# PacificBiosciences/trgt

Hardware: AMD Instinct MI355X
Metric: loci/s (higher is better)
Workload: dtype u8/u16 (WFA) + f64 (HMM); 1 GPU; BASELINE configs[1]: 10000 synthetic single-motif STR loci per GPU (motif 3-6 bp, allele <= 200 bp), 30 reads/locus HiFi-like, 10% truncated reads (SURVEY.md Appendix E), seed 20250509; contexts_per_gpu=4, loci_per_gpu=10000, reads_per_locus=30, parallelism=loci sharded across 1 GPU(s), no collective

## Files before the change

trgt_amd/csrc/common.hpp:

```cpp
#pragma once
#include <hip/hip_runtime.h>

#include <cstdarg>
#include <cstdint>
#include <cstdio>
#include <cstring>
#include <ctime>
#include <algorithm>
#include <mutex>
#include <string>
#include <vector>

#include "../../include/trgt_hip.h"

#ifdef TRGT_DEV_BUILD
#define TRGT_DEV_ENV(name) getenv(name)
#else
#define TRGT_DEV_ENV(name) ((const char*)nullptr)
#endif

struct trgt_knobs {
  int filter_force = 0;
  int flank_threads = 256;
  int heavy_band = 96;
  int heavy_threads = 0;
  int band_threads = 64;
  int win_threads = 64;
  int win_segments = 8;
  bool win_lds = false;
  int grid_per_cu = 0;
  int filter_per_cu = 0;
  bool one_launch = false;
  bool no_spec = false;
  bool no_window = false;
  bool early_adaptive = true;
  bool no_heavy_window = false;
  bool no_sibling_rule = false;
  bool no_settled_sibling_rule = false;
  bool no_lcs_rule = false;
  bool no_indel_shortcut = false;
  bool no_hamming = false;
  bool no_filter = false;
  bool one_stream = false;
  bool host_genotyper = false;
// ... 53 lines not shown
  uint64_t ws_limit = 32ull << 30;
  int32_t cluster_max_reads = 256;
  int32_t size_max_reads = 256;
  int64_t size_deep_stats[4] = {0, 0, 0, 0};
  bool flank_device = false;
  int64_t flank_stats[4] = {0, 0, 0, 0};
  bool snv_split_device = false;
  int64_t snv_split_stats[4] = {0, 0, 0, 0};
  bool flank_cluster_device = false;
  bool snv_cluster_device = false;
  int64_t snv_cluster_stats[4] = {0, 0, 0, 0};
  int64_t flank_cluster_stats[3] = {0, 0, 0};
  bool flank_cluster_deep_device = false;
  int64_t flank_cluster_deep_stats[3] = {0, 0, 0};
  int num_cus = 256;
  struct Buf { void* p = nullptr; size_t cap = 0; };
  std::vector<Buf> pool;
  bool timing = false;
  double k_ms[TRGT_K_COUNT] = {};
  int64_t k_launches[TRGT_K_COUNT] = {};
  int64_t k_cells[TRGT_K_COUNT] = {};
  struct Pending { int k; hipEvent_t a, b; };
  std::vector<Pending> pending;
  std::vector<hipEvent_t> retired_events;
  void* zero_arena = nullptr; size_t zero_cap = 0, zero_used = 0, zero_dirty = 0; bool zero_on = false;
  void* wfa_cells_cur[3] = {nullptr, nullptr, nullptr};
  void* last_wfa_cells_dev = nullptr;
  void* last_filter_cells_dev = nullptr;
  int64_t dbg_ns[8] = {0, 0, 0, 0, 0, 0, 0, 0};
  int64_t tl_t0 = 0;
// ... 115 lines not shown
  S_CL_VOUT, S_CL_VLEN, S_CL_VSCR,
  S_INF_SRC, S_INF_DESC, S_INF_DST, S_INF_STATUS, S_INF_COUNTER,
  S_ZERO_ARENA,
  S_DEFL_SCRATCH,
  S_PUR_SLAB, S_PUR_CNT, S_PUR_RQ,
  S_CLD_LIST, S_CLD_LAST = S_CLD_LIST + (S_CL_VSCR - S_CL_LIST),
  S_CLD_SEL,
  S_GSD_LIST,
  S_GT_HP,
  S_SNV_SO, S_SNV_EO, S_SNV_MM, S_SNV_MMOFF, S_SNV_READ,
  S_SNV_DEEP,
  S_CLF_COUNTS,
  S_CLF_PEND,
  S_CLDF_COUNTS, S_CLDF_PEND,
  S_FS_SETTLED, S_FS_FILTERJOBS,
  S_COUNT
};
enum PinSlot { P_SPAN_S = 0, P_SPAN_E, P_HIT_L, P_HIT_R, P_CELLS, P_HMM_SEQ, P_HMM_SEQ_B, P_HMM_JOBS, P_HMM_JOBS_B, P_SEG0, P_SEG_META, P_GT_NEED, P_GT_NAL, P_GT_ALEN, P_GT_CI, P_GT_NSP, P_GT_CLS,
               P_GT_RANK, P_GT_NSPAN, P_GT_TOFF, P_GT_PACKED, P_HMM_BUILD, P_PUR_JOBS, P_COUNT };

inline int dev_get(trgt_hip_ctx* c, int slot, size_t bytes, void** out) {
  if ((int)c->pool.size() < S_COUNT) c->pool.resize(S_COUNT);
  auto& b = c->pool[slot];
  if (bytes == 0) bytes = 16;
  if (b.cap < bytes) {
    if (b.p) { TRGT_HIP_TRY(c, hipFree(b.p)); b.p = nullptr; b.cap = 0; }
    size_t want = bytes + bytes / 8 + 256;
    if (c->knobs.debug && want > ((size_t)256 << 20)) fprintf(stderr, "[mem] slot %d: %.2f GB\n", slot, (double)want / (double)(1ull << 30));
    if (want >= ((size_t)64 << 20)) {
      size_t free_b = 0, total_b = 0;
// ... 298 lines not shown
```

trgt_amd/csrc/ctx.hip:

```cpp
#include "common.hpp"
#include "host_pool.hpp"

static std::string g_create_err;

#include <malloc.h>
static void tune_malloc_once() {
  static std::once_flag once;
  std::call_once(once, [] {
    const char* e = getenv("TRGT_MALLOC_TUNE");
    const int mode = e && *e ? atoi(e) : 1;
    if (mode <= 0) return;
    (void)mallopt(M_MMAP_THRESHOLD, 32 << 20);
    (void)mallopt(M_TRIM_THRESHOLD, 1 << 30);
    (void)mallopt(M_TOP_PAD, 64 << 20);
    if (mode >= 2) (void)mallopt(M_MMAP_MAX, 0);
  });
}

namespace trgt {
static thread_local int g_next_stream_priority = 0;
static thread_local bool g_next_in_pool = false;
void ctx_next_stream_priority(int p) { g_next_stream_priority = p; }
void ctx_next_in_pool(bool on) { g_next_in_pool = on; }
hipError_t make_stream(trgt_hip_ctx* c, hipStream_t* s) {
// ... 36 lines not shown
  tune_malloc_once();
  trgt_hip_ctx* c = new trgt_hip_ctx();
  {
    trgt_knobs& k = c->knobs;
    auto num = [](const char* name, int dflt) { const char* e = getenv(name); return e && *e ? atoi(e) : dflt; };
    auto flag = [](const char* name) { const char* e = getenv(name); return e != nullptr && *e != 0 && std::strcmp(e, "0") != 0; };
#ifdef TRGT_DEV_BUILD
#define DEV_FLAG(name) flag(name)
#define DEV_NUM(name, dflt) num(name, dflt)
#else
#define DEV_FLAG(name) false
#define DEV_NUM(name, dflt) (dflt)
#endif
    (void)num; (void)flag;
    k.flank_threads = DEV_NUM("TRGT_FLANK_THREADS", k.flank_threads); k.heavy_threads = DEV_NUM("TRGT_HEAVY_THREADS", 0); k.heavy_band = std::max(0, std::min(num("TRGT_HEAVY_BAND", k.heavy_band), 256));
    k.win_threads = DEV_NUM("TRGT_WIN_THREADS", k.win_threads); { const int bt = DEV_NUM("TRGT_BAND_THREADS", k.band_threads); k.band_threads = bt == 128 || bt == 256 ? bt : 64; } k.win_segments = DEV_NUM("TRGT_WIN_SEGMENTS", k.win_segments); k.win_lds = DEV_FLAG("TRGT_WIN_LDS");
    k.grid_per_cu = DEV_NUM("TRGT_WFA_GRID_PER_CU", 0); k.filter_per_cu = DEV_NUM("TRGT_FILTER_PER_CU", 0);
    k.one_launch = DEV_FLAG("TRGT_WFA_ONE_LAUNCH"); k.no_spec = DEV_FLAG("TRGT_WFA_NO_SPEC"); k.no_window = flag("TRGT_WFA_NO_WINDOW"); k.no_hamming = flag("TRGT_NO_HAMMING"); k.no_indel_shortcut = flag("TRGT_NO_INDEL_SHORTCUT"); k.no_heavy_window = DEV_FLAG("TRGT_NO_HEAVY_WINDOW"); k.no_sibling_rule = DEV_FLAG("TRGT_NO_SIBLING_RULE"); k.no_settled_sibling_rule = DEV_FLAG("TRGT_NO_SETTLED_SIBLING_RULE"); k.no_lcs_rule = DEV_FLAG("TRGT_NO_LCS_RULE"); { const char* e = TRGT_DEV_ENV("TRGT_EARLY_ADAPTIVE"); if (e && *e) k.early_adaptive = std::strcmp(e, "0") != 0; }
    k.no_filter = flag("TRGT_WFA_NO_FILTER"); k.one_stream = DEV_FLAG("TRGT_FLANK_ONE_STREAM"); k.host_genotyper = flag("TRGT_HOST_GENOTYPER"); k.host_hmm_lists = DEV_FLAG("TRGT_HOST_HMM_LISTS"); k.no_early = flag("TRGT_WFA_NO_EARLY"); k.stage_lock = flag("TRGT_STAGE_LOCK"); k.no_long_filter = flag("TRGT_NO_LONG_FILTER"); k.no_long_window = DEV_FLAG("TRGT_NO_LONG_WINDOW"); k.filter_force = DEV_NUM("TRGT_FILTER_FORCE", 0); k.filter_one_launch = DEV_FLAG("TRGT_FILTER_ONE_LAUNCH"); k.filter_serial = DEV_FLAG("TRGT_FILTER_SERIAL"); k.filter_side = DEV_FLAG("TRGT_FILTER_SIDE"); k.wfa_no_stage = DEV_FLAG("TRGT_WFA_NO_STAGE"); k.wfa_no_wave_variant = DEV_FLAG("TRGT_WFA_NO_WAVE_VARIANT"); k.hmm_resolve_one_wg = DEV_FLAG("TRGT_HMM_RESOLVE_ONE_WG"); k.debug = flag("TRGT_WFA_DEBUG");
    k.timeline = flag("TRGT_TIMELINE");
    k.host_repair = flag("TRGT_HOST_REPAIR"); k.host_cluster = flag("TRGT_HOST_CLUSTER"); k.host_purity = DEV_FLAG("TRGT_HOST_PURITY"); k.cluster_arena_kb = num("TRGT_CLUSTER_ARENA_KB", 0); k.repair_arena_kb = num("TRGT_REPAIR_ARENA_KB", 0); k.hmm_lds_fill = DEV_FLAG("TRGT_HMM_LDS_FILL"); k.hmm_four_rounds = DEV_FLAG("TRGT_HMM_FOUR_ROUNDS"); k.hmm_no_ppl = flag("TRGT_HMM_NO_PPL"); k.hmm_long_wgs = std::max(1, std::min(DEV_NUM("TRGT_HMM_LONG_WGS", k.hmm_long_wgs), 16)); k.hmm_no_long_tb = flag("TRGT_HMM_NO_LONG_TB"); k.hmm_no_dedupe = flag("TRGT_HMM_NO_DEDUPE"); k.repair_max_seg = num("TRGT_REPAIR_MAX_SEG", k.repair_max_seg); k.split_hmm = DEV_FLAG("TRGT_SPLIT_HMM"); k.repair_blocks = DEV_NUM("TRGT_REPAIR_BLOCKS", k.repair_blocks);
    k.no_lean = flag("TRGT_WFA_NO_LEAN"); k.lean_one_tier = DEV_FLAG("TRGT_WFA_LEAN_ONE_TIER"); k.lean_mid_tier = DEV_FLAG("TRGT_WFA_LEAN_MID_TIER"); k.lean_chunk = DEV_NUM("TRGT_LEAN_CHUNK", 0); k.no_zero_arena = flag("TRGT_NO_ZERO_ARENA"); k.hmm_ppl_serial = DEV_FLAG("TRGT_HMM_PPL_SERIAL"); k.hmm_ppl_wide = DEV_FLAG("TRGT_HMM_PPL_WIDE"); k.hmm_ppl_per_class = DEV_FLAG("TRGT_HMM_PPL_PER_CLASS");
    k.no_lds_wfa = !DEV_FLAG("TRGT_WFA_LDS"); k.lds_wfa_kb = DEV_NUM("TRGT_WFA_LDS_KB", k.lds_wfa_kb); k.lds_wfa_seq = DEV_NUM("TRGT_WFA_LDS_SEQ", k.lds_wfa_seq);
#ifdef TRGT_DEV_BUILD
    k.sens_bialign_min_len = num("TRGT_SENS_BIALIGN_MIN_LEN", -1); k.sens_cons_unidir = flag("TRGT_SENS_CONS_UNIDIR"); k.sens_ward_ties = flag("TRGT_SENS_WARD_TIES"); k.sens_lw_order = flag("TRGT_SENS_LW_ORDER");
    k.skip_bt = flag("TRGT_DBG_SKIP_BT");
#endif
  }
  c->device = device;
  c->num_cus = prop.multiProcessorCount;
  c->stream_priority = trgt::g_next_stream_priority;
// ... 106 lines not shown
```

trgt_amd/csrc/spans.hip:

```cpp
#include <algorithm>
#include <cmath>
#include <optional>

#include "wfa_host.hpp"

namespace trgt {

enum SpanCount : int {
  SC_HEAVY = 0,
  SC_LONG = 1,
  SC_LIGHT = 2,
  SC_ZERO = 3,
  SC_WIN = 4,
  SC_REST = 5,
  SC_KEEP = 6,
  SC_SHORTCUT = 7,
  SC_NOSEED = 8,
  SC_GAPS = 9,
  SC_BAND = 10,
  SC_HREST = 11,
  SC_BANDFAIL = 12,
  SC_LBAND = 13,
  SC_LREST = 14,
  SC_LNOSEED = 15,
  SC_SIBDROP = 16,
  SC_WINCLAIM = 17,
  SC_WINFALL = 18,
  SC_SETDROP = 19,
  SC_FILTER = 20,
  SC_LCSDROP = 21,
  SC_WORDS = 22
};

struct ScanArgs {
  const uint8_t* flank_blob; const uint8_t* read_blob;
  const uint64_t* piece_off;
  const uint64_t* read_off; const uint32_t* read_len; const uint32_t* read_locus;
  uint64_t n_jobs;
  int32_t flank_len;
  int32_t* pos;
  int32_t* n_match;
  JobDev* wfa_jobs; uint32_t* wfa_count;
  const uint32_t* heavy_len; uint32_t jobs_cap;
  JobDev* wfa_jobs_long; uint32_t long_tlen;
  int32_t min_matches;
  uint8_t* settled;
// ... 658 lines not shown
      a.kept[atomicAdd(a.n_kept, 1u)] = jd;
    }
}

struct SpanPlan {
  int64_t min_matches = 0; double threshold = 0; int32_t scan_min_matches = 0;
  int ring_slots = 0; uint32_t long_tlen = 0, short_max = 0, heavy_tlen_max = 0; bool has_long = false;
  int32_t win_m = WIN_SEGMENTS_DEFAULT, win_q = 0, win_s0 = 0, win_margin = 0, win_spread = 0, win_tbf = 0; uint32_t win_tlen = 0;
  int32_t hamming_max = 0, indel_ok = 0; bool win_reg = false;
  bool split = false, use_filter = false, two_streams = false; int64_t flt_tlen = 0;
  bool heavy_window = false;
  bool settled_rule = false;
  int32_t lcs_max_adm = 0;
  bool sibling_pass = false;
  bool heavy_band = false;
  bool long_window = false;
  bool long_filter = false, long_band = false; int64_t long_wl = 0, long_step = 0; uint64_t long_cap = 0;
  int flank_threads = 0, heavy_threads = 0, win_threads = 0, band_threads = 0, band_s_max = 0; bool early_reject = false, count_offsets = false;
};
static SpanPlan span_plan(const trgt_hip_ctx* c, const trgt_span_params& p, uint64_t n_jobs, uint32_t max_read_len, uint32_t heavy_tlen_max, bool have_heavy_len, bool span_only) {
  const trgt_knobs& k = c->knobs;
  const bool wgs = preset_wgs(p.mism, p.gapo, p.gape), filter_pen = preset_has_filter(p.mism, p.gapo, p.gape);
  SpanPlan P;
  const double thr = (double)(uint64_t)p.flank_len * p.min_flank_id_frac;
  int64_t min_matches = thr > 0 ? (int64_t)std::ceil(thr) : 0;
  while (min_matches > 0 && (double)(min_matches - 1) >= thr) --min_matches;
  while ((double)min_matches < thr) ++min_matches;
  P.min_matches = min_matches; P.threshold = thr;
  P.scan_min_matches = span_only && !k.no_sibling_rule ? (int32_t)std::min<int64_t>(min_matches, 0x7FFFFFFF) : 0;
  P.ring_slots = std::max(p.mism, p.gapo + p.gape) + 1 + 2 * (p.gape + 1);
// ... 9 lines not shown
  const int q = p.flank_len / m, x = p.mism, o = p.gapo, e = p.gape;
  if (P.split && !k.no_window && q >= 12 && x >= 1 && e >= 1 && o >= 0 && q * e >= x && o + 2 * e >= 2 * x && o + e >= x) {
    P.win_s0 = x * m - 1;
    const int G = P.win_s0 >= o + e ? (P.win_s0 - o) / e : 0, C = P.win_s0 / e;
    P.win_q = q; P.win_margin = G + C; P.win_spread = 2 * G;
    P.win_tlen = (uint32_t)(p.flank_len + 2 * P.win_margin + P.win_spread);
    if (P.win_tlen + 64 >= max_read_len) P.win_q = 0;
  }
  if (P.win_q > 0) {
    P.win_tbf = 2 * P.win_margin + P.win_spread;
    P.hamming_max = k.no_hamming ? 0 : std::min(std::min(P.win_m - 1, (p.gapo + p.gape - 1) / p.mism), 4);
    P.indel_ok = !k.no_hamming && !k.no_indel_shortcut && wgs && P.hamming_max == 2 ? 1 : 0;
    P.win_reg = !k.win_lds && !k.skip_bt && !k.no_spec && wfa_win_fits(p.mism, p.gapo, p.gape, P.win_tbf, P.win_s0, p.flank_len, P.win_tlen);
  }
  const bool band_ok = k.heavy_band > 0 && wgs && !k.no_spec && !k.skip_bt && !k.wfa_no_stage;
  if (P.split) {
    P.flt_tlen = flank_filter_max_tlen(p.flank_len);
    P.use_filter = filter_pen && P.flt_tlen >= 2 * (int64_t)p.flank_len &&
                   P.heavy_tlen_max >= (uint32_t)p.flank_len && min_matches <= 254 && !k.no_filter;
    P.two_streams = P.use_filter && !k.one_stream;
    P.heavy_window = P.use_filter && P.two_streams && P.win_q > 0 && !k.no_heavy_window;
    P.settled_rule = P.heavy_window && P.scan_min_matches > 0 && P.hamming_max > 0 && !k.no_settled_sibling_rule;
    P.lcs_max_adm = P.heavy_window && P.scan_min_matches > 0 && p.flank_len <= LCS_MAX_F && !k.no_lcs_rule ? LCS_MAX_ADM : 0;
    P.sibling_pass = P.settled_rule || P.lcs_max_adm > 0;
    P.heavy_band = P.use_filter && band_ok;
  }
  P.long_window = P.has_long && P.win_q > 0 && !k.no_long_window;
  if (P.has_long) {
    const int64_t wl = flank_filter_max_tlen(p.flank_len);
    const int64_t span_max = 2 * (int64_t)p.flank_len + p.gapo + 8, step = wl - span_max;
// ... 20 lines not shown
};
struct SpanCall {
  trgt_hip_ctx* const c; const trgt_span_params& p; const int64_t n_reads; const uint64_t n_jobs;
  const uint8_t* d_flank; const uint64_t* d_piece_off; const uint8_t* d_reads; const uint64_t* d_read_off; const uint32_t* d_read_len; const uint32_t* d_read_locus;
  const uint32_t max_read_len; int32_t* d_span_start; int32_t* d_span_end; uint8_t* d_lf_hit; uint8_t* d_rf_hit; const uint32_t* d_heavy_len;
  const SpanPlan plan;
  JobDev *wjobs = nullptr, *wjobs_long = nullptr, *winjobs = nullptr, *restjobs = nullptr, *long_noseed = nullptr;
  uint32_t *count = nullptr, *span4 = nullptr; int32_t *pos = nullptr, *nmatch = nullptr, *score = nullptr;
  uint8_t* settled = nullptr;
  trgt_wfa_params wp; WfaLaunch heavy, light, longl;
  JobList long_in{nullptr, nullptr};
  bool set_started[2] = {false, false}; void* heavy_cells = nullptr;
  template <class T> int get(int slot, size_t bytes, T*& out) { void* v = nullptr; const int rc = dev_get(c, slot, bytes, &v); out = (T*)v; return rc; }
  int seed_search(bool front, JobDev* rest, JobDev* long_rest);
  int band_backtrace(JobList& list, int slot_band, int slot_rest, int slot_score, int i_band, int i_rest, const WfaLaunch& base, int buffer_set);
  int launch(const trgt_wfa_params& wpl, WfaLaunch L) {
    bool& started = set_started[L.buffer_set ? 1 : 0];
    L.keep_cells = started; started = true;
    return wfa_launch(c, wpl, L);
  }
  int first_launch_done() {
    if (plan.two_streams) { heavy_cells = c->last_wfa_cells_dev; return TRGT_OK; }
    TRGT_HIP_TRY(c, hipMemcpyAsync((uint8_t*)c->last_wfa_cells_dev + 8, c->last_wfa_cells_dev, 8, hipMemcpyDeviceToDevice, c->stream));
    return TRGT_OK;
  }
  int merge_cells() {
    hipLaunchKernelGGL(cells_merge_kernel, dim3(1), dim3(1), 0, c->stream, (unsigned long long*)c->last_wfa_cells_dev, (const unsigned long long*)heavy_cells);
    TRGT_HIP_TRY(c, hipGetLastError());
    return TRGT_OK;
  }
// ... 51 lines not shown
  wa.flank_blob = d_flank; wa.read_blob = d_reads; wa.wfa_jobs = wjobs; wa.jobs_cap = (uint32_t)n_jobs; wa.count = count;
  wa.win_jobs = winjobs; wa.rest_jobs = rest; wa.flank_len = p.flank_len; wa.q = plan.win_q; wa.margin = plan.win_margin; wa.spread = plan.win_spread; wa.tbf = plan.win_tbf;
  wa.front = front ? 1 : 0; wa.long_jobs = long_rest ? wjobs_long : nullptr; wa.long_rest = long_rest;
  wa.hamming_max = plan.hamming_max; wa.indel_ok = plan.indel_ok;
  wa.n_match = nmatch; wa.span4 = span4; wa.settled = front ? settled : nullptr;
  KTimer t(c, TRGT_K_FLANK_WINDOW);
  const dim3 wgrid((unsigned)std::max<int64_t>(1, std::min<int64_t>((int64_t)c->num_cus * 8, (int64_t)((n_jobs + WIN_JOBS_PER_WG - 1) / WIN_JOBS_PER_WG))));
  if (plan.win_m == 4) hipLaunchKernelGGL(flank_window_kernel<4>, wgrid, dim3(256), 0, c->stream, wa);
  else if (plan.win_m == 6) hipLaunchKernelGGL(flank_window_kernel<6>, wgrid, dim3(256), 0, c->stream, wa);
  else hipLaunchKernelGGL(flank_window_kernel<8>, wgrid, dim3(256), 0, c->stream, wa);
  TRGT_HIP_TRY(c, hipGetLastError());
  t.stop(0);
  return TRGT_OK;
}
int SpanCall::band_backtrace(JobList& list, int slot_band, int slot_rest, int slot_score, int i_band, int i_rest, const WfaLaunch& base, int buffer_set) {
  int rc; JobDev *band = nullptr, *rest = nullptr; int32_t* bscore = nullptr;
  if ((rc = get(slot_band, n_jobs * sizeof(JobDev), band)) || (rc = get(slot_rest, n_jobs * sizeof(JobDev), rest)) || (rc = get(slot_score, n_jobs * 4, bscore)))
    return rc;
  const int s_max = plan.band_s_max;
  BandArgs ba;
  ba.keep_jobs = list.jobs; ba.n_keep = list.count; ba.band_jobs = band; ba.rest_jobs = rest; ba.count = count;
  ba.s_max = s_max; ba.score = bscore; ba.span4 = span4; ba.n_match = nmatch;
  ba.read_off = d_read_off; ba.read_len = d_read_len; ba.i_band = i_band; ba.i_rest = i_rest;
  hipLaunchKernelGGL(heavy_band_kernel, dim3(64), dim3(256), 0, c->stream, ba);
  TRGT_HIP_TRY(c, hipGetLastError());
  WfaLaunch LB = base;
  LB.jobs_dev = band; LB.n_jobs_dev = count + i_band;
  LB.max_tlen = (int64_t)p.flank_len + 2 * s_max; LB.max_sum = (int64_t)p.flank_len + LB.max_tlen;
  LB.score = bscore; LB.kernel_tag = 3; LB.max_score = s_max; LB.threads = plan.band_threads; LB.buffer_set = buffer_set;
  trgt_wfa_params wpb = wp;
  wpb.text_begin_free = 2 * s_max;
  if ((rc = launch(wpb, LB))) return rc;
  hipLaunchKernelGGL(band_check_kernel, dim3(64), dim3(256), 0, c->stream, ba);
  TRGT_HIP_TRY(c, hipGetLastError());
  list = {rest, count + i_rest};
  return TRGT_OK;
}
int SpanCall::heavy_list() {
  int rc;
  std::optional<OnStream2> on_stream2;
  if (plan.two_streams) {
    if (!c->stream2) TRGT_HIP_TRY(c, trgt::make_stream(c, &c->stream2));
    if (!c->ev_scan) TRGT_HIP_TRY(c, hipEventCreateWithFlags(&c->ev_scan, hipEventDisableTiming));
    if (!c->ev_heavy) TRGT_HIP_TRY(c, hipEventCreateWithFlags(&c->ev_heavy, hipEventDisableTiming));
    TRGT_HIP_TRY(c, hipEventRecord(c->ev_scan, c->stream));
    TRGT_HIP_TRY(c, hipStreamWaitEvent(c->stream2, c->ev_scan, 0));
    on_stream2.emplace(c);
  }
  JobList list{wjobs, count + SC_HEAVY};
  if (plan.heavy_window) {
// ... 121 lines not shown
  hipLaunchKernelGGL(span_combine_kernel, dim3((unsigned)((n_reads + 255) / 256)), dim3(256), 0, c->stream, ca);
  TRGT_HIP_TRY(c, hipGetLastError());
  return TRGT_OK;
}
int SpanCall::debug_report() {
  uint32_t h[SC_WORDS];
  TRGT_HIP_TRY(c, trgt::stream_wait(c, c->stream));
  TRGT_HIP_TRY(c, hipMemcpy(h, count, 4 * SC_WORDS, hipMemcpyDeviceToHost));
  const bool win = plan.win_q > 0;
  if (win)
    fprintf(stderr, "[spans] fallback alignments: first launch %u, long reads %u, light %u -> windowed %u, whole read %u (that is %u without seeds + %u windows that did not stand), settled by the shortcuts %u (one-base gaps: %u)\n",
            h[SC_HEAVY], h[SC_LONG], h[SC_LIGHT], h[SC_WIN], h[SC_REST], h[SC_LIGHT] - h[SC_WIN] - h[SC_SHORTCUT], h[SC_REST] - (h[SC_LIGHT] - h[SC_WIN] - h[SC_SHORTCUT]), h[SC_SHORTCUT], h[SC_GAPS]);
  if (!win) fprintf(stderr, "[spans] fallback alignments: first launch %u, long reads %u, light %u (no seeded windows for this configuration)\n", h[SC_HEAVY], h[SC_LONG], h[SC_LIGHT]);
  if (win) fprintf(stderr, "[spans+] windowed launch: %s, %u alignments it did not take\n", plan.win_reg ? "one wave per alignment, history in registers" : "LDS kernel", h[SC_WINFALL]);
  if (win && plan.heavy_window) fprintf(stderr, "[spans+] (the seed search ran over the first launch's list too: %u of its %u alignments had no seeds and met the pre-filter; the counts of the windowed list and of the shortcut include the others)\n", h[SC_NOSEED], h[SC_HEAVY]);
  if (plan.has_long) fprintf(stderr, "[spans+] long reads kept by the window filter: back-traced inside a band %u, over the whole read %u\n", h[SC_LBAND], h[SC_LREST]);
  fprintf(stderr, "[spans+] sibling rule %s: %u missed pieces without a job (fewer than %d bases beside the exactly found sibling)\n", plan.scan_min_matches > 0 ? "on" : "off", h[SC_SIBDROP], plan.scan_min_matches);
  if (win && plan.heavy_window) fprintf(stderr, "[spans+] settled-sibling rule %s: %u jobs without seeds never met the pre-filter (fewer than %d bases beside a sibling the shortcuts settled)\n", plan.settled_rule ? "on" : "off", h[SC_SETDROP], plan.scan_min_matches);
  if (win && plan.heavy_window) fprintf(stderr, "[spans+] common-subsequence rule %s: %u jobs without seeds never met the pre-filter (no common subsequence of %d bases with the %d to %d bases beside a sibling found exactly or settled by the shortcuts); %u met it\n", plan.lcs_max_adm > 0 ? "on" : "off", h[SC_LCSDROP], plan.scan_min_matches, plan.scan_min_matches, plan.lcs_max_adm, plan.sibling_pass ? h[SC_FILTER] : h[SC_NOSEED]);
  if (plan.heavy_band) fprintf(stderr, "[spans+] kept by the pre-filter: %u -> back-traced inside a band %u (did not stand: %u), over the whole read %u\n", h[SC_KEEP], h[SC_BAND], h[SC_BANDFAIL], h[SC_HREST]);
  return TRGT_OK;
}

int find_spans_device(trgt_hip_ctx* c, const trgt_span_params& p, int64_t n_reads, const uint8_t* d_flank, const uint64_t* d_piece_off,
                      const uint8_t* d_reads, const uint64_t* d_read_off, const uint32_t* d_read_len, const uint32_t* d_read_locus,
                      uint32_t max_read_len, int32_t* d_span_start, int32_t* d_span_end, uint8_t* d_lf_hit, uint8_t* d_rf_hit,
                      const uint32_t* d_heavy_len, uint32_t heavy_tlen_max, bool span_only) {
  const uint64_t n_jobs = 2ull * (uint64_t)n_reads;
  SpanCall s{c, p, n_reads, n_jobs, d_flank, d_piece_off, d_reads, d_read_off, d_read_len, d_read_locus, max_read_len, d_span_start, d_span_end, d_lf_hit, d_rf_hit, d_heavy_len,
             span_plan(c, p, n_jobs, max_read_len, heavy_tlen_max, d_heavy_len != nullptr, span_only)};
  int rc;
  if ((rc = s.workspace()) || (rc = s.scan())) return rc;
  if (s.plan.split && (rc = s.heavy_list())) return rc;
  if (s.plan.win_q > 0 && (rc = s.light_windows())) return rc;
  if ((rc = s.rest_launch())) return rc;
// ... 74 lines not shown
```

trgt_amd/csrc/wfa_host.hpp:

```cpp
#pragma once
#include <functional>
#include <vector>
#include "common.hpp"

namespace trgt {

struct JobDev {
  uint64_t pat_off, txt_off, cigar_off, ops_off;
  uint32_t pat_len, txt_len, out_index, pad;
};


inline uint32_t heavy_read_len(uint32_t locus_max_read_len, int flank_len) {
  const uint32_t margin = (uint32_t)flank_len + (uint32_t)flank_len / 5;
  return locus_max_read_len > margin ? locus_max_read_len - margin : 0;
}

inline bool preset_wgs(int mism, int gapo, int gape) { return mism == 2 && gapo == 5 && gape == 1; }
inline bool preset_has_filter(int mism, int gapo, int gape) { return preset_wgs(mism, gapo, gape) || (mism == 1 && gapo == 0 && gape == 1); }

struct WfaLaunch {
  const JobDev* jobs_dev = nullptr; int64_t n_jobs_host = 0; const uint32_t* n_jobs_dev = nullptr;
  int64_t jobs_bound = 0;
  const uint32_t* n_jobs2_dev = nullptr; uint32_t jobs_cap = 0;
// ... 13 lines not shown

int wfa_launch(trgt_hip_ctx* c, const trgt_wfa_params& p, const WfaLaunch& L);

struct WfaWinLaunch {
  const JobDev* jobs_dev = nullptr; int64_t n_jobs_host = 0; const uint32_t* n_jobs_dev = nullptr;
  const uint8_t* pat_base = nullptr; const uint8_t* txt_base = nullptr;
  int tbf = 0, s_max = 0;
  unsigned int* counter = nullptr;
  unsigned int* fallback = nullptr;
  int32_t* score = nullptr; int32_t* n_match = nullptr; uint32_t* span4 = nullptr;
  int timer_slot = TRGT_K_WFA_FLANK_REST;
};
bool wfa_win_fits(int mism, int gapo, int gape, int tbf, int s_max, int64_t max_plen, int64_t max_tlen);
int wfa_win_launch(trgt_hip_ctx* c, const WfaWinLaunch& L);

int wfa_lean_launch(trgt_hip_ctx* c, const trgt_wfa_params& p, const WfaLaunch& L, JobDev* mid_jobs, JobDev* retry_jobs, unsigned int* retry_count, uint32_t retry_cap,
                    unsigned int* retry_lost, unsigned int* counters, unsigned long long* cells_out, unsigned int* why_hist);

struct FilterArgs {
  const JobDev* jobs; const uint32_t* n_jobs_dev; uint32_t n_jobs;
  const uint8_t* pat_base; const uint8_t* txt_base;
  unsigned int* counter;
  int32_t min_matches;
  int32_t early_reject;
  JobDev* keep_jobs; uint32_t* keep_count;
  int32_t* score; int32_t* bound; uint8_t* keep;
  uint32_t* band;
  int32_t diag_lo, diag_hi;
  unsigned long long* cells_out;
};
// ... 32 lines not shown
```

Before: 4.534 million loci/s.

## Add register-resident one-wave banded WFA kernel for flank back-trace jobs

Adds a new banded WFA kernel that runs one 64-lane wave per alignment. It keeps the wavefront history in registers, uses DPP lane shifts for neighbouring diagonals, and records span endpoints while running forward, so no back-trace is needed. Jobs whose band or pattern exceeds the register caps are routed to the existing LDS heavy-band path. The intent is to drop the LDS-heavy band kernel, its extra launches and its check kernel for most banded jobs. In exchange it adds register pressure, fallback bookkeeping and a second code path that must give the same spans.

New measurement: 4.795 million loci/s (median of 6 runs). 1.06x the previous value.

```diff
diff --git a/trgt_amd/csrc/common.hpp b/trgt_amd/csrc/common.hpp
--- a/trgt_amd/csrc/common.hpp
+++ b/trgt_amd/csrc/common.hpp
@@ -28,6 +28,7 @@
   int win_threads = 64;
   int win_segments = 8;
   bool win_lds = false;
+  bool band_lds = false;
   int grid_per_cu = 0;
   int filter_per_cu = 0;
   bool one_launch = false;
@@ -111,6 +112,7 @@
   bool flank_cluster_deep_device = false;
   int64_t flank_cluster_deep_stats[3] = {0, 0, 0};
   int num_cus = 256;
+  int band_occ = 0;
   struct Buf { void* p = nullptr; size_t cap = 0; };
   std::vector<Buf> pool;
   bool timing = false;
@@ -256,6 +258,7 @@
   S_CLF_PEND,
   S_CLDF_COUNTS, S_CLDF_PEND,
   S_FS_SETTLED, S_FS_FILTERJOBS,
+  S_FS_BANDFALL, S_LW_BANDFALL,
   S_COUNT
 };
 enum PinSlot { P_SPAN_S = 0, P_SPAN_E, P_HIT_L, P_HIT_R, P_CELLS, P_HMM_SEQ, P_HMM_SEQ_B, P_HMM_JOBS, P_HMM_JOBS_B, P_SEG0, P_SEG_META, P_GT_NEED, P_GT_NAL, P_GT_ALEN, P_GT_CI, P_GT_NSP, P_GT_CLS,
diff --git a/trgt_amd/csrc/ctx.hip b/trgt_amd/csrc/ctx.hip
--- a/trgt_amd/csrc/ctx.hip
+++ b/trgt_amd/csrc/ctx.hip
@@ -74,7 +74,7 @@
 #endif
     (void)num; (void)flag;
     k.flank_threads = DEV_NUM("TRGT_FLANK_THREADS", k.flank_threads); k.heavy_threads = DEV_NUM("TRGT_HEAVY_THREADS", 0); k.heavy_band = std::max(0, std::min(num("TRGT_HEAVY_BAND", k.heavy_band), 256));
-    k.win_threads = DEV_NUM("TRGT_WIN_THREADS", k.win_threads); { const int bt = DEV_NUM("TRGT_BAND_THREADS", k.band_threads); k.band_threads = bt == 128 || bt == 256 ? bt : 64; } k.win_segments = DEV_NUM("TRGT_WIN_SEGMENTS", k.win_segments); k.win_lds = DEV_FLAG("TRGT_WIN_LDS");
+    k.win_threads = DEV_NUM("TRGT_WIN_THREADS", k.win_threads); { const int bt = DEV_NUM("TRGT_BAND_THREADS", k.band_threads); k.band_threads = bt == 128 || bt == 256 ? bt : 64; } k.win_segments = DEV_NUM("TRGT_WIN_SEGMENTS", k.win_segments); k.win_lds = DEV_FLAG("TRGT_WIN_LDS"); k.band_lds = DEV_FLAG("TRGT_BAND_LDS");
     k.grid_per_cu = DEV_NUM("TRGT_WFA_GRID_PER_CU", 0); k.filter_per_cu = DEV_NUM("TRGT_FILTER_PER_CU", 0);
     k.one_launch = DEV_FLAG("TRGT_WFA_ONE_LAUNCH"); k.no_spec = DEV_FLAG("TRGT_WFA_NO_SPEC"); k.no_window = flag("TRGT_WFA_NO_WINDOW"); k.no_hamming = flag("TRGT_NO_HAMMING"); k.no_indel_shortcut = flag("TRGT_NO_INDEL_SHORTCUT"); k.no_heavy_window = DEV_FLAG("TRGT_NO_HEAVY_WINDOW"); k.no_sibling_rule = DEV_FLAG("TRGT_NO_SIBLING_RULE"); k.no_settled_sibling_rule = DEV_FLAG("TRGT_NO_SETTLED_SIBLING_RULE"); k.no_lcs_rule = DEV_FLAG("TRGT_NO_LCS_RULE"); { const char* e = TRGT_DEV_ENV("TRGT_EARLY_ADAPTIVE"); if (e && *e) k.early_adaptive = std::strcmp(e, "0") != 0; }
     k.no_filter = flag("TRGT_WFA_NO_FILTER"); k.one_stream = DEV_FLAG("TRGT_FLANK_ONE_STREAM"); k.host_genotyper = flag("TRGT_HOST_GENOTYPER"); k.host_hmm_lists = DEV_FLAG("TRGT_HOST_HMM_LISTS"); k.no_early = flag("TRGT_WFA_NO_EARLY"); k.stage_lock = flag("TRGT_STAGE_LOCK"); k.no_long_filter = flag("TRGT_NO_LONG_FILTER"); k.no_long_window = DEV_FLAG("TRGT_NO_LONG_WINDOW"); k.filter_force = DEV_NUM("TRGT_FILTER_FORCE", 0); k.filter_one_launch = DEV_FLAG("TRGT_FILTER_ONE_LAUNCH"); k.filter_serial = DEV_FLAG("TRGT_FILTER_SERIAL"); k.filter_side = DEV_FLAG("TRGT_FILTER_SIDE"); k.wfa_no_stage = DEV_FLAG("TRGT_WFA_NO_STAGE"); k.wfa_no_wave_variant = DEV_FLAG("TRGT_WFA_NO_WAVE_VARIANT"); k.hmm_resolve_one_wg = DEV_FLAG("TRGT_HMM_RESOLVE_ONE_WG"); k.debug = flag("TRGT_WFA_DEBUG");
diff --git a/trgt_amd/csrc/spans.hip b/trgt_amd/csrc/spans.hip
--- a/trgt_amd/csrc/spans.hip
+++ b/trgt_amd/csrc/spans.hip
@@ -29,7 +29,11 @@
   SC_SETDROP = 19,
   SC_FILTER = 20,
   SC_LCSDROP = 21,
-  SC_WORDS = 22
+  SC_BANDCLAIM = 22,
+  SC_BANDFALL = 23,
+  SC_BANDREG = 24,
+  SC_LBANDCLAIM = 25, SC_LBANDFALL = 26, SC_LBANDREG = 27,
+  SC_WORDS = 28
 };
 
 struct ScanArgs {
@@ -718,6 +722,7 @@
   int32_t lcs_max_adm = 0;
   bool sibling_pass = false;
   bool heavy_band = false;
+  bool band_reg = false;
   bool long_window = false;
   bool long_filter = false, long_band = false; int64_t long_wl = 0, long_step = 0; uint64_t long_cap = 0;
   int flank_threads = 0, heavy_threads = 0, win_threads = 0, band_threads = 0, band_s_max = 0; bool early_reject = false, count_offsets = false;
@@ -757,6 +762,7 @@
     P.win_reg = !k.win_lds && !k.skip_bt && !k.no_spec && wfa_win_fits(p.mism, p.gapo, p.gape, P.win_tbf, P.win_s0, p.flank_len, P.win_tlen);
   }
   const bool band_ok = k.heavy_band > 0 && wgs && !k.no_spec && !k.skip_bt && !k.wfa_no_stage;
+  P.band_reg = band_ok && !k.band_lds;
   if (P.split) {
     P.flt_tlen = flank_filter_max_tlen(p.flank_len);
     P.use_filter = filter_pen && P.flt_tlen >= 2 * (int64_t)p.flank_len &&
@@ -807,6 +813,7 @@
   template <class T> int get(int slot, size_t bytes, T*& out) { void* v = nullptr; const int rc = dev_get(c, slot, bytes, &v); out = (T*)v; return rc; }
   int seed_search(bool front, JobDev* rest, JobDev* long_rest);
   int band_backtrace(JobList& list, int slot_band, int slot_rest, int slot_score, int i_band, int i_rest, const WfaLaunch& base, int buffer_set);
+  int band_lds_launches(const JobList& kept, JobDev* rest, int slot_band, int slot_score, int i_band, int i_rest, const WfaLaunch& base, int buffer_set);
   int launch(const trgt_wfa_params& wpl, WfaLaunch L) {
     bool& started = set_started[L.buffer_set ? 1 : 0];
     L.keep_cells = started; started = true;
@@ -888,12 +895,34 @@
   return TRGT_OK;
 }
 int SpanCall::band_backtrace(JobList& list, int slot_band, int slot_rest, int slot_score, int i_band, int i_rest, const WfaLaunch& base, int buffer_set) {
-  int rc; JobDev *band = nullptr, *rest = nullptr; int32_t* bscore = nullptr;
-  if ((rc = get(slot_band, n_jobs * sizeof(JobDev), band)) || (rc = get(slot_rest, n_jobs * sizeof(JobDev), rest)) || (rc = get(slot_score, n_jobs * 4, bscore)))
-    return rc;
+  int rc; JobDev* rest = nullptr;
+  if ((rc = get(slot_rest, n_jobs * sizeof(JobDev), rest))) return rc;
+  const int s_max = plan.band_s_max;
+  if (plan.band_reg) {
+    const bool short_list = i_band == SC_BAND;
+    const bool may_fall = s_max > WFA_BAND_S_CAP || p.flank_len > WFA_BAND_PLEN_MAX;
+    JobDev* fall = nullptr;
+    if (may_fall && (rc = get(short_list ? S_FS_BANDFALL : S_LW_BANDFALL, n_jobs * sizeof(JobDev), fall))) return rc;
+    WfaBandLaunch BL;
+    BL.jobs_dev = list.jobs; BL.n_jobs_host = (int64_t)n_jobs; BL.n_jobs_dev = list.count; BL.pat_base = d_flank; BL.txt_base = d_reads;
+    BL.count = count; BL.i_claim = short_list ? SC_BANDCLAIM : SC_LBANDCLAIM; BL.i_reg = BL.i_claim + 2; BL.i_fall = BL.i_claim + 1;
+    BL.i_rest = i_rest; BL.i_fail = SC_BANDFAIL; BL.fall_jobs = fall; BL.rest_jobs = rest;
+    BL.n_match = nmatch; BL.span4 = span4; BL.read_off = d_read_off; BL.read_len = d_read_len; BL.s_max = s_max; BL.timer_slot = base.timer_slot;
+    if ((rc = wfa_band_launch(c, BL))) return rc;
+    list = {rest, count + i_rest};
+    if (!may_fall) return TRGT_OK;
+    return band_lds_launches(JobList{fall, count + BL.i_fall}, rest, slot_band, slot_score, i_band, i_rest, base, buffer_set);
+  }
+  if ((rc = band_lds_launches(list, rest, slot_band, slot_score, i_band, i_rest, base, buffer_set))) return rc;
+  list = {rest, count + i_rest};
+  return TRGT_OK;
+}
+int SpanCall::band_lds_launches(const JobList& kept, JobDev* rest, int slot_band, int slot_score, int i_band, int i_rest, const WfaLaunch& base, int buffer_set) {
+  int rc; JobDev* band = nullptr; int32_t* bscore = nullptr;
+  if ((rc = get(slot_band, n_jobs * sizeof(JobDev), band)) || (rc = get(slot_score, n_jobs * 4, bscore))) return rc;
   const int s_max = plan.band_s_max;
   BandArgs ba;
-  ba.keep_jobs = list.jobs; ba.n_keep = list.count; ba.band_jobs = band; ba.rest_jobs = rest; ba.count = count;
+  ba.keep_jobs = kept.jobs; ba.n_keep = kept.count; ba.band_jobs = band; ba.rest_jobs = rest; ba.count = count;
   ba.s_max = s_max; ba.score = bscore; ba.span4 = span4; ba.n_match = nmatch;
   ba.read_off = d_read_off; ba.read_len = d_read_len; ba.i_band = i_band; ba.i_rest = i_rest;
   hipLaunchKernelGGL(heavy_band_kernel, dim3(64), dim3(256), 0, c->stream, ba);
@@ -907,7 +936,6 @@
   if ((rc = launch(wpb, LB))) return rc;
   hipLaunchKernelGGL(band_check_kernel, dim3(64), dim3(256), 0, c->stream, ba);
   TRGT_HIP_TRY(c, hipGetLastError());
-  list = {rest, count + i_rest};
   return TRGT_OK;
 }
 int SpanCall::heavy_list() {
@@ -1059,11 +1087,12 @@
   if (!win) fprintf(stderr, "[spans] fallback alignments: first launch %u, long reads %u, light %u (no seeded windows for this configuration)\n", h[SC_HEAVY], h[SC_LONG], h[SC_LIGHT]);
   if (win) fprintf(stderr, "[spans+] windowed launch: %s, %u alignments it did not take\n", plan.win_reg ? "one wave per alignment, history in registers" : "LDS kernel", h[SC_WINFALL]);
   if (win && plan.heavy_window) fprintf(stderr, "[spans+] (the seed search ran over the first launch's list too: %u of its %u alignments had no seeds and met the pre-filter; the counts of the windowed list and of the shortcut include the others)\n", h[SC_NOSEED], h[SC_HEAVY]);
-  if (plan.has_long) fprintf(stderr, "[spans+] long reads kept by the window filter: back-traced inside a band %u, over the whole read %u\n", h[SC_LBAND], h[SC_LREST]);
+  if (plan.has_long) fprintf(stderr, "[spans+] long reads kept by the window filter: back-traced inside a band %u, over the whole read %u\n", h[SC_LBAND] + h[SC_LBANDREG], h[SC_LREST]);
   fprintf(stderr, "[spans+] sibling rule %s: %u missed pieces without a job (fewer than %d bases beside the exactly found sibling)\n", plan.scan_min_matches > 0 ? "on" : "off", h[SC_SIBDROP], plan.scan_min_matches);
   if (win && plan.heavy_window) fprintf(stderr, "[spans+] settled-sibling rule %s: %u jobs without seeds never met the pre-filter (fewer than %d bases beside a sibling the shortcuts settled)\n", plan.settled_rule ? "on" : "off", h[SC_SETDROP], plan.scan_min_matches);
   if (win && plan.heavy_window) fprintf(stderr, "[spans+] common-subsequence rule %s: %u jobs without seeds never met the pre-filter (no common subsequence of %d bases with the %d to %d bases beside a sibling found exactly or settled by the shortcuts); %u met it\n", plan.lcs_max_adm > 0 ? "on" : "off", h[SC_LCSDROP], plan.scan_min_matches, plan.scan_min_matches, plan.lcs_max_adm, plan.sibling_pass ? h[SC_FILTER] : h[SC_NOSEED]);
-  if (plan.heavy_band) fprintf(stderr, "[spans+] kept by the pre-filter: %u -> back-traced inside a band %u (did not stand: %u), over the whole read %u\n", h[SC_KEEP], h[SC_BAND], h[SC_BANDFAIL], h[SC_HREST]);
+  if (plan.heavy_band) fprintf(stderr, "[spans+] kept by the pre-filter: %u -> back-traced inside a band %u (did not stand: %u), over the whole read %u\n", h[SC_KEEP], h[SC_BAND] + h[SC_BANDREG], h[SC_BANDFAIL], h[SC_HREST]);
+  if (plan.heavy_band || plan.long_band) fprintf(stderr, "[spans+] banded launch: %s, %u + %u alignments left to the LDS kernel\n", plan.band_reg ? "one wave per alignment, forward only" : "LDS kernel", h[SC_BANDFALL], h[SC_LBANDFALL]);
   return TRGT_OK;
 }
 
diff --git a/trgt_amd/csrc/wfa_band.hip b/trgt_amd/csrc/wfa_band.hip
--- /dev/null
+++ b/trgt_amd/csrc/wfa_band.hip
@@ -0,0 +1,296 @@
+#include "wfa_host.hpp"
+
+namespace trgt {
+namespace {
+
+constexpr int BAND_NPL = 7;
+constexpr int BAND_CAP = WFA_BAND_S_CAP;
+constexpr int BAND_PLEN_MAX = WFA_BAND_PLEN_MAX;
+constexpr int BAND_SEQ_DW = 132;
+static_assert(4 * BAND_CAP + 1 <= 64 * BAND_NPL, "the band of the highest penalty must fit the lanes");
+static_assert(BAND_PLEN_MAX + 2 * BAND_CAP <= 504, "the window of the highest penalty must fit the staging buffer");
+static_assert(64 * BAND_NPL <= 512 && BAND_PLEN_MAX <= 255, "summary fields: 9-bit diagonals, 8-bit pattern positions");
+
+struct BandKArgs {
+  const JobDev* jobs; const uint32_t* n_jobs_dev;
+  const uint8_t* pat_base; const uint8_t* txt_base;
+  uint32_t* count; int32_t i_claim, i_reg, i_fall, i_rest, i_fail;
+  JobDev* fall_jobs; JobDev* rest_jobs;
+  int32_t* n_match; uint32_t* span4;
+  const uint64_t* read_off; const uint32_t* read_len;
+  int32_t s_max;
+};
+
+constexpr uint32_t B_PE = 0xFFu, B_KL = 0x1FFu << 17, B_STARTED = 1u << 26;
+
+__device__ __forceinline__ uint32_t band_ffbl(uint32_t v) {
+  uint32_t r;
+  asm("v_ffbl_b32 %0, %1" : "=v"(r) : "v"(v));
+  return r;
+}
+__device__ __forceinline__ uint32_t band_below(uint32_t x) { return (uint32_t)__builtin_amdgcn_update_dpp(0, (int)x, 0x138 , 0xF, 0xF, false); }
+__device__ __forceinline__ uint32_t band_above(uint32_t x) { return (uint32_t)__builtin_amdgcn_update_dpp(0, (int)x, 0x130 , 0xF, 0xF, false); }
+__device__ __forceinline__ int band_rfl(int v) { return __builtin_amdgcn_readfirstlane(v); }
+__device__ __forceinline__ uint32_t band_enc(uint32_t a) { return a & 0xFFFFu; }
+
+__device__ __forceinline__ uint32_t band_window(const uint32_t* S, int i) {
+  const int d = i >> 2;
+  return __builtin_amdgcn_alignbyte(S[d + 1], S[d], (uint32_t)i & 3u);
+}
+__device__ __forceinline__ void band_stage(const uint8_t* __restrict__ src, int len, uint32_t* S, int lane) {
+  const int i0 = 8 * lane;
+  uint64_t w = 0;
+  if (i0 + 8 <= len) __builtin_memcpy(&w, src + i0, 8);
+  else if (i0 < len) {
+    if (len >= 8) { __builtin_memcpy(&w, src + len - 8, 8); w >>= 8 * (8 - (len - i0)); }
+    else for (int b = 0; b < len; ++b) w |= (uint64_t)src[b] << (8 * b);
+  }
+  S[2 * lane] = (uint32_t)w; S[2 * lane + 1] = (uint32_t)(w >> 32);
+  if (lane < BAND_SEQ_DW - 128) S[128 + lane] = 0u;
+}
+
+struct BandEnd { int s; uint32_t a, b; };
+template <int NPL>
+__device__ __forceinline__ BandEnd band_run(const uint32_t* Pq, const uint32_t* Tq, const int lane, const int plen, const int tlen, const int tbf, const int s_star,
+                                            const int kbase) {
+  int end_s = -1; uint32_t end_a = 0, end_b = 0;
+  int ln = lane;
+  asm volatile("" : "+v"(ln));
+  const int kA = kbase + NPL * ln, kbA = NPL * ln;
+  auto step4 = [&](int v, int h) -> uint32_t {
+    const uint32_t xw = band_window(Pq, v) ^ band_window(Tq, h);
+    return min(min(band_ffbl(xw) >> 3, 4u), (uint32_t)min(plen - v, tlen - h));
+  };
+  auto finish_runs = [&](bool c, int& v, int& h) {
+    unsigned long long m = __ballot(c);
+    while (m) {
+      const int jl = (int)__builtin_ctzll(m);
+      m &= m - 1ull;
+      int vj = __builtin_amdgcn_readlane(v, jl), hj = __builtin_amdgcn_readlane(h, jl);
+      for (;;) {
+        const int pv = vj + 4 * lane, ph = hj + 4 * lane;
+        const int rem = min(plen - pv, tlen - ph);
+        const uint32_t xw = band_window(Pq, min(pv, plen)) ^ band_window(Tq, min(ph, tlen));
+        const uint32_t n = rem > 0 ? min(min(band_ffbl(xw) >> 3, 4u), (uint32_t)rem) : 0u;
+        const unsigned long long stop = __ballot(n < 4u);
+        if (stop) {
+          const int js = (int)__builtin_ctzll(stop);
+          const int ext = 4 * js + __builtin_amdgcn_readlane((int)n, js);
+          vj += ext; hj += ext;
+          break;
+        }
+        vj += 256; hj += 256;
+      }
+      if (lane == jl) { v = vj; h = hj; }
+    }
+  };
+  auto extend_cells = [&](uint32_t (&pa)[NPL], uint32_t (&pb)[NPL], bool (&term)[NPL]) -> bool {
+    int v[NPL], h[NPL], h0[NPL];
+    bool ok[NPL], c[NPL];
+    bool any = false;
+#pragma unroll
+    for (int d = 0; d < NPL; ++d) {
+      const int k = kA + d, hp = (int)band_enc(pa[d]) - 1, vp = hp - k;
+      ok[d] = (uint32_t)hp <= (uint32_t)tlen && (uint32_t)vp <= (uint32_t)plen;
+      v[d] = ok[d] ? vp : 0; h[d] = ok[d] ? hp : 0; h0[d] = h[d];
+      const uint32_t n = step4(v[d], h[d]);
+      v[d] += (int)n; h[d] += (int)n;
+      c[d] = ok[d] && n == 4u;
+      any = any || c[d];
+    }
+    if (__ballot(any)) {
+#pragma unroll
+      for (int d = 0; d < NPL; ++d) {
+        if (c[d]) { const uint32_t n = step4(v[d], h[d]); v[d] += (int)n; h[d] += (int)n; c[d] = n == 4u; }
+        finish_runs(c[d], v[d], h[d]);
+      }
+    }
+    bool t = false;
+#pragma unroll
+    for (int d = 0; d < NPL; ++d) {
+      const uint32_t kb = (uint32_t)(kbA + d), ext = (uint32_t)(h[d] - h0[d]);
+      uint32_t qa = (pa[d] & 0xFFFF0000u) + (ext << 16) + (uint32_t)h[d] + 1u, qb = pb[d];
+      if (ext) {
+        if (!(qb & B_STARTED)) { qa = (qa & 0x00FFFFFFu) | ((uint32_t)(v[d] - (int)ext) << 24); qb = (kb << 8) | B_STARTED; }
+        qb = (qb & ~(B_PE | B_KL)) | (uint32_t)v[d] | (kb << 17);
+      }
+      pa[d] = ok[d] ? qa : 0u; pb[d] = ok[d] ? qb : 0u;
+      term[d] = ok[d] && v[d] >= plen;
+      t = t || term[d];
+    }
+    return t;
+  };
+  auto trim = [&](uint32_t (&xa)[NPL], uint32_t (&xb)[NPL]) {
+    int fd = NPL, ld = -1;
+#pragma unroll
+    for (int d = NPL - 1; d >= 0; --d) {
+      const uint32_t e = band_enc(xa[d]) - 1u;
+      const bool in = e <= (uint32_t)tlen && (e - (uint32_t)(kA + d)) <= (uint32_t)plen;
+      fd = in ? d : fd; ld = in && ld < 0 ? d : ld;
+    }
+    const unsigned long long bl = __ballot(fd < NPL);
+    int first = 64 * NPL, last = -1;
+    if (bl) {
+      const int fl = (int)__builtin_ctzll(bl), ll = 63 - (int)__builtin_clzll(bl);
+      first = NPL * fl + __builtin_amdgcn_readlane(fd, fl); last = NPL * ll + __builtin_amdgcn_readlane(ld, ll);
+    }
+#pragma unroll
+    for (int d = 0; d < NPL; ++d) {
+      const bool keep = kbA + d >= first && kbA + d <= last;
+      xa[d] = keep ? xa[d] : 0u; xb[d] = keep ? xb[d] : 0u;
+    }
+  };
+  auto terminated = [&](int s, bool t, const uint32_t (&pa)[NPL], const uint32_t (&pb)[NPL], const bool (&term)[NPL]) {
+    const unsigned long long tb = __ballot(t);
+    if (!tb) return;
+    uint32_t ta = 0, tq = 0;
+#pragma unroll
+    for (int d = NPL - 1; d >= 0; --d) { ta = term[d] ? pa[d] : ta; tq = term[d] ? pb[d] : tq; }
+    const int l = (int)__builtin_ctzll(tb);
+    end_a = (uint32_t)__builtin_amdgcn_readlane((int)ta, l); end_b = (uint32_t)__builtin_amdgcn_readlane((int)tq, l);
+    end_s = s;
+  };
+
+  uint32_t Ma[6][NPL], Mb[6][NPL], Ia[NPL], Ib[NPL], Da[NPL], Db[NPL];
+#pragma unroll
+  for (int d = 0; d < NPL; ++d) {
+#pragma unroll
+    for (int r = 0; r < 6; ++r) { Ma[r][d] = 0u; Mb[r][d] = 0u; }
+    Ia[d] = 0u; Ib[d] = 0u; Da[d] = 0u; Db[d] = 0u;
+  }
+#pragma nounroll
+  for (int s = 0; s <= s_star && end_s < 0; ++s) {
+    uint32_t gIa[NPL], gIb[NPL], gDa[NPL], gDb[NPL];
+#pragma unroll
+    for (int d = 0; d < NPL; ++d) {
+      const uint32_t mo = band_enc(Ma[5][d]);
+      const bool ti = band_enc(Ia[d]) >= mo, td = band_enc(Da[d]) >= mo;
+      gIa[d] = ti ? Ia[d] : Ma[5][d]; gIb[d] = ti ? Ib[d] : Mb[5][d];
+      gDa[d] = td ? Da[d] : Ma[5][d]; gDb[d] = td ? Db[d] : Mb[5][d];
+    }
+    const uint32_t belowA = band_below(gIa[NPL - 1]), belowB = band_below(gIb[NPL - 1]);
+    const uint32_t aboveA = band_above(gDa[0]), aboveB = band_above(gDb[0]);
+    uint32_t pa[NPL], pb[NPL];
+    bool term[NPL];
+#pragma unroll
+    for (int d = 0; d < NPL; ++d) {
+      const int k = kA + d;
+      const uint32_t kb = (uint32_t)(kbA + d);
+      uint32_t ia = d ? gIa[d - 1] : belowA, ib = d ? gIb[d - 1] : belowB;
+      uint32_t da = d < NPL - 1 ? gDa[d + 1] : aboveA, db = d < NPL - 1 ? gDb[d + 1] : aboveB;
+      ia += min(band_enc(ia), 1u);
+      { const int hh = (int)band_enc(ia) - 1, vv = hh - k; if (hh <= 0 || vv <= 0) { ia &= 0xFFFFu; ib = 0u; } }
+      { const int hh = (int)band_enc(da) - 1, vv = hh - k; if (hh <= 0 || vv <= 0) { da &= 0xFFFFu; db = 0u; } }
+      Ia[d] = ia; Ib[d] = ib; Da[d] = da; Db[d] = db;
+      uint32_t xa = Ma[1][d], xb = Mb[1][d];
+      if (band_enc(xa)) {
+        xa += 1u;
+        const uint32_t vv = band_enc(xa) - 1u - (uint32_t)k;
+        if (!(xb & B_STARTED)) { xa = (xa & 0x00FFFFFFu) | ((vv - 1u) << 24); xb = (kb << 8) | B_STARTED; }
+        xb = (xb & ~(B_PE | B_KL)) | vv | (kb << 17);
+      }
+      const bool dwin = band_enc(da) >= band_enc(ia);
+      uint32_t qa = dwin ? da : ia, qb = dwin ? db : ib;
+      const bool xwin = band_enc(xa) >= band_enc(qa);
+      pa[d] = xwin ? xa : qa; pb[d] = xwin ? xb : qb;
+      if (s == 0) { pa[d] = k >= 0 && k <= tbf ? (uint32_t)k + 1u : 0u; pb[d] = 0u; }
+    }
+    const bool t = extend_cells(pa, pb, term);
+    trim(Ia, Ib); trim(Da, Db);
+    terminated(s, t, pa, pb, term);
+#pragma unroll
+    for (int d = 0; d < NPL; ++d) {
+#pragma unroll
+      for (int r = 5; r >= 1; --r) { Ma[r][d] = Ma[r - 1][d]; Mb[r][d] = Mb[r - 1][d]; }
+      Ma[0][d] = pa[d]; Mb[0][d] = pb[d];
+    }
+  }
+  BandEnd E;
+  E.s = end_s; E.a = end_a; E.b = end_b;
+  return E;
+}
+
+__device__ __forceinline__ void band_hand_on(JobDev* dst, const JobDev* src, uint64_t txt_off, uint32_t txt_len, uint32_t pad, uint32_t out_index) {
+  dst->pat_off = src->pat_off; dst->txt_off = txt_off; dst->cigar_off = 0; dst->ops_off = 0;
+  dst->pat_len = src->pat_len; dst->txt_len = txt_len; dst->out_index = out_index; dst->pad = pad;
+}
+
+__global__ void __launch_bounds__(64, 2) wfa_band_kernel(const BandKArgs a) {
+  __shared__ uint32_t lds_seq[2 * BAND_SEQ_DW];
+  uint32_t* const Pq = lds_seq;
+  uint32_t* const Tq = lds_seq + BAND_SEQ_DW;
+  const int lane = threadIdx.x;
+  const uint32_t n_jobs = *a.n_jobs_dev;
+  uint32_t n_taken = 0;
+  for (;;) {
+    uint32_t jc = 0;
+    if (lane == 0) jc = atomicAdd(a.count + a.i_claim, 1u);
+    const uint32_t j = (uint32_t)band_rfl((int)jc);
+    if (j >= n_jobs) break;
+    const JobDev* const job = a.jobs + j;
+    const uint32_t pad = (uint32_t)band_rfl((int)job->pad), o = (uint32_t)band_rfl((int)job->out_index);
+    const int plen = band_rfl((int)job->pat_len), rlen = band_rfl((int)job->txt_len);
+    const int s_star = (int)((pad >> 16) & 0x7FFFu), k_end = (int)(pad & 0xFFFFu) - plen;
+    const int t0 = max(0, k_end - s_star), k_hi = min(k_end + s_star, rlen), t_end = min(rlen, k_end + s_star + plen);
+    if (!((pad >> 31) && s_star <= a.s_max && k_hi >= t0 && t_end > t0)) {
+      if (lane == 0) band_hand_on(a.rest_jobs + atomicAdd(a.count + a.i_rest, 1u), job, job->txt_off, job->txt_len, 0u, o);
+      continue;
+    }
+    if (s_star > BAND_CAP || plen > BAND_PLEN_MAX) {
+      if (lane == 0) { JobDev* const dst = a.fall_jobs + atomicAdd(a.count + a.i_fall, 1u); band_hand_on(dst, job, job->txt_off, job->txt_len, pad, o); dst->cigar_off = job->cigar_off; dst->ops_off = job->ops_off; }
+      continue;
+    }
+    ++n_taken;
+    const int tlen = t_end - t0, tbf = k_hi - t0;
+    band_stage(a.pat_base + job->pat_off, plen, Pq, lane);
+    band_stage(a.txt_base + job->txt_off + (uint64_t)t0, tlen, Tq, lane);
+    asm volatile("" ::: "memory");
+
+    const int kbase = -s_star, width = tbf + 2 * s_star + 1;
+    BandEnd E;
+    if (width <= 128) E = band_run<2>(Pq, Tq, lane, plen, tlen, tbf, s_star, kbase);
+    else if (width <= 256) E = band_run<4>(Pq, Tq, lane, plen, tlen, tbf, s_star, kbase);
+    else if (width <= 384) E = band_run<6>(Pq, Tq, lane, plen, tlen, tbf, s_star, kbase);
+    else E = band_run<BAND_NPL>(Pq, Tq, lane, plen, tlen, tbf, s_star, kbase);
+    const int end_s = E.s; const uint32_t end_a = E.a, end_b = E.b;
+    const int nm = (int)((end_a >> 16) & 0xFFu);
+    if (lane == 0) {
+      if (end_s == s_star && nm > 0) {
+        const uint32_t ps = end_a >> 24, pe = end_b & B_PE;
+        const int kf = (int)((end_b >> 8) & 0x1FFu) + kbase, kl = (int)((end_b >> 17) & 0x1FFu) + kbase;
+        a.n_match[o] = nm;
+        *reinterpret_cast<uint4*>(a.span4 + 4 * (size_t)o) = make_uint4(ps, pe, (uint32_t)((int)ps + kf + t0), (uint32_t)((int)pe + kl + t0));
+      } else {
+        a.n_match[o] = -1;
+        band_hand_on(a.rest_jobs + atomicAdd(a.count + a.i_rest, 1u), job, a.read_off[o >> 1], a.read_len[o >> 1], 0u, o);
+        atomicAdd(a.count + a.i_fail, 1u);
+      }
+    }
+  }
+  if (lane == 0 && n_taken) atomicAdd(a.count + a.i_reg, n_taken);
+}
+
+}
+
+int wfa_band_launch(trgt_hip_ctx* c, const WfaBandLaunch& L) {
+  BandKArgs a;
+  a.jobs = L.jobs_dev; a.n_jobs_dev = L.n_jobs_dev; a.pat_base = L.pat_base; a.txt_base = L.txt_base;
+  a.count = L.count; a.i_claim = L.i_claim; a.i_reg = L.i_reg; a.i_fall = L.i_fall; a.i_rest = L.i_rest; a.i_fail = L.i_fail;
+  a.fall_jobs = L.fall_jobs; a.rest_jobs = L.rest_jobs; a.n_match = L.n_match; a.span4 = L.span4;
+  a.read_off = L.read_off; a.read_len = L.read_len; a.s_max = L.s_max;
+  if (c->band_occ < 1) {
+    int occ = 0;
+    if (hipOccupancyMaxActiveBlocksPerMultiprocessor(&occ, wfa_band_kernel, 64, 0) != hipSuccess || occ < 1) { (void)hipGetLastError(); occ = 8; }
+    c->band_occ = std::min(occ, 16);
+  }
+  const int occ = c->band_occ;
+  const int64_t grid = std::max<int64_t>(1, std::min<int64_t>((int64_t)c->num_cus * occ, L.n_jobs_host));
+  if (c->knobs.debug) fprintf(stderr, "[wfa] banded launch in registers: occupancy=%d grid=%lld\n", occ, (long long)grid);
+  KTimer t(c, L.timer_slot);
+  hipLaunchKernelGGL(wfa_band_kernel, dim3((unsigned)grid), dim3(64), 0, c->stream, a);
+  TRGT_HIP_TRY(c, hipGetLastError());
+  t.stop(0);
+  return TRGT_OK;
+}
+
+}
diff --git a/trgt_amd/csrc/wfa_host.hpp b/trgt_amd/csrc/wfa_host.hpp
--- a/trgt_amd/csrc/wfa_host.hpp
+++ b/trgt_amd/csrc/wfa_host.hpp
@@ -51,6 +51,20 @@
 bool wfa_win_fits(int mism, int gapo, int gape, int tbf, int s_max, int64_t max_plen, int64_t max_tlen);
 int wfa_win_launch(trgt_hip_ctx* c, const WfaWinLaunch& L);
 
+constexpr int WFA_BAND_S_CAP = 96, WFA_BAND_PLEN_MAX = 255;
+struct WfaBandLaunch {
+  const JobDev* jobs_dev = nullptr; int64_t n_jobs_host = 0; const uint32_t* n_jobs_dev = nullptr;
+  const uint8_t* pat_base = nullptr; const uint8_t* txt_base = nullptr;
+  uint32_t* count = nullptr;
+  int i_claim = 0, i_reg = 0, i_fall = 0, i_rest = 0, i_fail = 0;
+  JobDev* fall_jobs = nullptr; JobDev* rest_jobs = nullptr;
+  int32_t* n_match = nullptr; uint32_t* span4 = nullptr;
+  const uint64_t* read_off = nullptr; const uint32_t* read_len = nullptr;
+  int s_max = 0;
+  int timer_slot = TRGT_K_WFA_FLANK;
+};
+int wfa_band_launch(trgt_hip_ctx* c, const WfaBandLaunch& L);
+
 int wfa_lean_launch(trgt_hip_ctx* c, const trgt_wfa_params& p, const WfaLaunch& L, JobDev* mid_jobs, JobDev* retry_jobs, unsigned int* retry_count, uint32_t retry_cap,
                     unsigned int* retry_lost, unsigned int* counters, unsigned long long* cells_out, unsigned int* why_hist);
 
```
